# alpc91/SGRL

Hardware: AMD Instinct MI355X
Metric: env-steps/sec (whole node) + SET-actor fwd us/step, 3d_walker mix @8192 envs/GPU (higher is better)
Workload: dtype f64 (dynamics) / f32 (SET actor, obs); 1 GPU; 3D_Walker++ 8 variants x 1024 envs per GPU (config 3), random U(-1,1) actions, auto-reset, SET actor forward on every step, random-init weights; envs_per_gpu=8192, obs_max_len=287, action_max_len=21, replay_gather=none (single rank)

## Files before the change

include/sgrl_model.h:

```cpp
#ifndef SGRL_MODEL_H
#define SGRL_MODEL_H

#include <stdint.h>

#ifdef __HIPCC__
#define SGRL_HD __host__ __device__ inline
#else
#define SGRL_HD static inline
#endif

#define SGRL_MAGIC 0x5347524C
#define SGRL_MAXDEPTH 8

enum {
  SGRL_H_MAGIC = 0,
  SGRL_H_NBODY,
  SGRL_H_NJNT,
  SGRL_H_NQ,
  SGRL_H_NV,
  SGRL_H_NU,
  SGRL_H_NGEOM,
  SGRL_H_NPAIR,
  SGRL_H_INTEGRATOR,
  SGRL_H_FRAME_SKIP,
  SGRL_H_DONE_RULE,
  SGRL_H_TARGET_V2,
  SGRL_H_RESET_VEL_NORMAL,
  SGRL_H_NHEIGHT_BODIES,
  SGRL_H_HEIGHT_BODY0,
  SGRL_H_HEIGHT_BODY1,
  SGRL_H_MAX_ROWS,
  SGRL_H_PGS_ITERS,
  SGRL_H_SOLVER,
  SGRL_NHDR = 24
};

enum {
  SGRL_F_TIMESTEP = 0,
  SGRL_F_GRAV_X, SGRL_F_GRAV_Y, SGRL_F_GRAV_Z,
  SGRL_F_HEIGHT_LO, SGRL_F_HEIGHT_HI, SGRL_F_ANG_LIMIT,
  SGRL_F_ALIVE_BONUS, SGRL_F_HEADING_WEIGHT, SGRL_F_CTRL_COST,
  SGRL_F_RESET_POS_NOISE, SGRL_F_RESET_VEL_NOISE,
  SGRL_F_PGS_TOL,
  SGRL_F_TOTAL_MASS,
  SGRL_NFHDR = 16
};

enum {
  SGRL_RC_DMIN = 0, SGRL_RC_DMAX, SGRL_RC_WIDTH, SGRL_RC_MID, SGRL_RC_POWER,
  SGRL_RC_K, SGRL_RC_B, SGRL_RC_MARGIN, SGRL_RC_MU, SGRL_RC_TRAN, SGRL_RC_RF1, SGRL_RC_RF2,
  SGRL_ROWC = 12
};

enum { SGRL_GEOM_PLANE = 0, SGRL_GEOM_SPHERE = 2, SGRL_GEOM_CAPSULE = 3 };
enum { SGRL_JNT_FREE = 0, SGRL_JNT_HINGE = 3 };

#ifndef SGRL_CONST_AS
#define SGRL_CONST_AS
#endif
#ifndef SGRL_ITAB_AS
#define SGRL_ITAB_AS
#endif
#ifndef SGRL_FTAB_AS
#define SGRL_FTAB_AS
#endif
typedef const SGRL_CONST_AS int32_t* sgrl_hdr_t;
typedef const SGRL_CONST_AS double* sgrl_fhdr_t;
typedef const SGRL_ITAB_AS int32_t* sgrl_itab_t;
typedef const SGRL_FTAB_AS double* sgrl_ftab_t;

typedef struct SgrlModelView {
  sgrl_hdr_t hdr;
  sgrl_fhdr_t fhdr;
  int nbody, njnt, nq, nv, nu, ngeom, npair;
  sgrl_itab_t body_parent, body_jntadr, body_jntnum, body_dofadr, body_dofnum, body_limbtype;
  sgrl_itab_t jnt_type, jnt_body, jnt_qposadr, jnt_dofadr, jnt_limited;
  sgrl_itab_t dof_body, dof_jnt, dof_parent;
  sgrl_itab_t geom_type, geom_body;
  sgrl_itab_t pair_g1, pair_g2, pair_condim;
  sgrl_itab_t act_dof, act_slot;
  sgrl_itab_t body_depth;
  sgrl_itab_t body_path;
  sgrl_itab_t body_subend;
  sgrl_itab_t body_dofmask;
  sgrl_itab_t dof_act;
  sgrl_ftab_t qpos0;
  sgrl_ftab_t body_pos, body_quat, body_ipos, body_inertia, body_mass, body_invweight0;
  sgrl_ftab_t jnt_pos, jnt_axis, jnt_range, jnt_stiffness, jnt_solref, jnt_solimp, jnt_margin;
  sgrl_ftab_t dof_armature, dof_damping, dof_invweight0;
  sgrl_ftab_t geom_pos, geom_quat, geom_size;
  sgrl_ftab_t pair_mu, pair_margin, pair_solref, pair_solimp;
  sgrl_ftab_t act_gear, act_ctrlrange;
  sgrl_ftab_t geom_axis;
  sgrl_ftab_t pair_rowc;
  sgrl_ftab_t jnt_rowc;
  int n_int, n_f64;
} SgrlModelView;

SGRL_HD int sgrl_model_view_dims(const int32_t* dims, sgrl_hdr_t hdr_src, sgrl_fhdr_t fhdr_src, sgrl_itab_t ib, sgrl_ftab_t fb,
                                 SgrlModelView* v) {
  if (dims[SGRL_H_MAGIC] != SGRL_MAGIC) return -1;
  v->hdr = hdr_src;
  v->fhdr = fhdr_src;
  const int nb = dims[SGRL_H_NBODY], nj = dims[SGRL_H_NJNT], nq = dims[SGRL_H_NQ], nv = dims[SGRL_H_NV];
  const int nu = dims[SGRL_H_NU], ng = dims[SGRL_H_NGEOM], np = dims[SGRL_H_NPAIR];
  v->nbody = nb; v->njnt = nj; v->nq = nq; v->nv = nv; v->nu = nu; v->ngeom = ng; v->npair = np;
  sgrl_itab_t p = ib + SGRL_NHDR;
  v->body_parent = p; p += nb;
  v->body_jntadr = p; p += nb;
  v->body_jntnum = p; p += nb;
  v->body_dofadr = p; p += nb;
  v->body_dofnum = p; p += nb;
  v->body_limbtype = p; p += nb;
  v->jnt_type = p; p += nj;
  v->jnt_body = p; p += nj;
  v->jnt_qposadr = p; p += nj;
  v->jnt_dofadr = p; p += nj;
  v->jnt_limited = p; p += nj;
// ... 71 lines not shown
```

sgrl_amd/csrc/step_body.h:

```cpp
#pragma once

#include <math.h>
#include <stdint.h>

#include "../../include/sgrl_model.h"

#ifdef __HIPCC__
#define SGRL_DEV __device__ __forceinline__
#else
#define SGRL_DEV inline
#endif

namespace sgrl {

constexpr double kMinVal = 1e-15;
constexpr double kMinImp = 0.0001;
constexpr double kMaxImp = 0.9999;
constexpr double kPi = 3.14159265358979323846;
constexpr int kNAMax = 32;
constexpr int kBppMaxIter = 40;
constexpr int kSlabRows = 256;
constexpr int kPivotRows = 64;
constexpr int kPrevRows = 48;
constexpr int kSlabLdy = 47;
// ... 183 lines not shown
SGRL_DEV void quat2mat(double* m, const double* q) {
  const double q00 = q[0] * q[0], q11 = q[1] * q[1], q22 = q[2] * q[2], q33 = q[3] * q[3];
  m[0] = q00 + q11 - q22 - q33; m[4] = q00 - q11 + q22 - q33; m[8] = q00 - q11 - q22 + q33;
  m[1] = 2 * (q[1] * q[2] - q[0] * q[3]); m[2] = 2 * (q[1] * q[3] + q[0] * q[2]);
  m[3] = 2 * (q[1] * q[2] + q[0] * q[3]); m[5] = 2 * (q[2] * q[3] - q[0] * q[1]);
  m[6] = 2 * (q[1] * q[3] - q[0] * q[2]); m[7] = 2 * (q[2] * q[3] + q[0] * q[1]);
}
SGRL_DEV void mat_vec(double* r, const double* m, const double* v) {
  const double x = m[0] * v[0] + m[1] * v[1] + m[2] * v[2];
  const double y = m[3] * v[0] + m[4] * v[1] + m[5] * v[2];
  const double z = m[6] * v[0] + m[7] * v[1] + m[8] * v[2];
  r[0] = x; r[1] = y; r[2] = z;
}
SGRL_DEV void axisangle2quat(double* q, const double* axis, double angle) {
  if (angle == 0.0) { q[0] = 1; q[1] = 0; q[2] = 0; q[3] = 0; return; }
  double s, c;
  sincos(0.5 * angle, &s, &c);
  q[0] = c; q[1] = axis[0] * s; q[2] = axis[1] * s; q[3] = axis[2] * s;
}
SGRL_DEV void inert_mul(double* f, const double* I, const double* mv) {
  const double* w = mv; const double* v = mv + 3; const double* h = I + 6;
  double hv[3], hw[3];
  cross3(hv, h, v); cross3(hw, h, w);
  f[0] = I[0] * w[0] + I[3] * w[1] + I[4] * w[2] + hv[0];
  f[1] = I[3] * w[0] + I[1] * w[1] + I[5] * w[2] + hv[1];
  f[2] = I[4] * w[0] + I[5] * w[1] + I[2] * w[2] + hv[2];
  f[3] = I[9] * v[0] - hw[0]; f[4] = I[9] * v[1] - hw[1]; f[5] = I[9] * v[2] - hw[2];
}
SGRL_DEV void cross_motion(double* r, const double* vel, const double* m) {
  double a[3], b[3], c[3];
  cross3(a, vel, m); cross3(b, vel, m + 3); cross3(c, vel + 3, m);
  r[0] = a[0]; r[1] = a[1]; r[2] = a[2];
  r[3] = b[0] + c[0]; r[4] = b[1] + c[1]; r[5] = b[2] + c[2];
}
SGRL_DEV void cross_force(double* r, const double* vel, const double* f) {
  double a[3], b[3], c[3];
  cross3(a, vel, f); cross3(b, vel + 3, f + 3); cross3(c, vel, f + 3);
  r[0] = a[0] + b[0]; r[1] = a[1] + b[1]; r[2] = a[2] + b[2];
  r[3] = c[0]; r[4] = c[1]; r[5] = c[2];
}
SGRL_DEV void ld3(double* r, const double* p) { r[0] = p[0]; r[1] = p[1]; r[2] = p[2]; }
SGRL_DEV void ld6(double* r, const double* p) { r[0] = p[0]; r[1] = p[1]; r[2] = p[2]; r[3] = p[3]; r[4] = p[4]; r[5] = p[5]; }
SGRL_DEV int popcount64(uint64_t x) {
#ifdef __HIPCC__
  return __popcll(x);
#else
  return __builtin_popcountll(x);
#endif
}
SGRL_DEV int clz64(uint64_t x) {
#ifdef __HIPCC__
  return __clzll((long long)x);
#else
  return __builtin_clzll(x);
#endif
}
SGRL_DEV int tri(int i) { return i * (i + 1) / 2; }
SGRL_DEV void tri_decode(int p, int* a_out, int* b_out) {
  int a = (int)((sqrtf(8.0f * (float)p + 1.0f) - 1.0f) * 0.5f);
  a += ((a + 1) * (a + 2) / 2 <= p) ? 1 : 0;
  a -= (a * (a + 1) / 2 > p) ? 1 : 0;
  *a_out = a; *b_out = p - a * (a + 1) / 2;
}
SGRL_DEV bool dof_in_mask(sgrl_itab_t mask2, int d) {
  const uint32_t w = (uint32_t)(d < 32 ? mask2[0] : mask2[1]);
  return (w >> (d & 31)) & 1u;
}

SGRL_DEV double rng_uniform01(uint64_t seed, uint32_t env_id, uint32_t episode, uint32_t stream, uint32_t idx) {
  uint32_t c0 = idx >> 2, c1 = episode, c2 = stream, c3 = (uint32_t)(seed >> 32);
  uint32_t k0 = (uint32_t)seed, k1 = env_id;
  for (int r = 0; r < 10; r++) {
    const uint64_t p0 = (uint64_t)0xD2511F53u * c0, p1 = (uint64_t)0xCD9E8D57u * c2;
    const uint32_t n0 = (uint32_t)(p1 >> 32) ^ c1 ^ k0, n1 = (uint32_t)p1;
    const uint32_t n2 = (uint32_t)(p0 >> 32) ^ c3 ^ k1, n3 = (uint32_t)p0;
    c0 = n0; c1 = n1; c2 = n2; c3 = n3;
    k0 += 0x9E3779B9u; k1 += 0xBB67AE85u;
  }
  const uint32_t lane = idx & 3u;
  const uint32_t x = lane == 0 ? c0 : (lane == 1 ? c1 : (lane == 2 ? c2 : c3));
  return ((double)x + 0.5) * (1.0 / 4294967296.0);
}

#ifdef SGRL_PHASE_PROF
#define SGRL_TICK(id) w.tick(id)
#else
#define SGRL_TICK(id)
#endif

template <class W>
struct Engine {
  W& w;
  SgrlModelView m;
  const Layout& o;
  double* S;
  int32_t* I;
  double* big_scratch = nullptr;
  bool linv = false;

  SGRL_DEV Engine(W& w_, const SgrlModelView& m_, const Layout& o_, double* S_, int32_t* I_)
      : w(w_), m(m_), o(o_), S(S_), I(I_) {}

  SGRL_DEV void fence_view() {
    if (W::kFixedDims) return;
    m.body_parent = w.fenced(m.body_parent); m.body_jntadr = w.fenced(m.body_jntadr);
    m.body_jntnum = w.fenced(m.body_jntnum); m.body_dofadr = w.fenced(m.body_dofadr);
    m.body_dofnum = w.fenced(m.body_dofnum); m.body_limbtype = w.fenced(m.body_limbtype);
    m.jnt_type = w.fenced(m.jnt_type); m.jnt_body = w.fenced(m.jnt_body);
    m.jnt_qposadr = w.fenced(m.jnt_qposadr); m.jnt_dofadr = w.fenced(m.jnt_dofadr);
    m.jnt_limited = w.fenced(m.jnt_limited); m.dof_body = w.fenced(m.dof_body); m.dof_jnt = w.fenced(m.dof_jnt);
    m.dof_parent = w.fenced(m.dof_parent); m.geom_type = w.fenced(m.geom_type);
    m.geom_body = w.fenced(m.geom_body); m.pair_g1 = w.fenced(m.pair_g1); m.pair_g2 = w.fenced(m.pair_g2);
    m.pair_condim = w.fenced(m.pair_condim); m.act_dof = w.fenced(m.act_dof); m.act_slot = w.fenced(m.act_slot);
    m.body_depth = w.fenced(m.body_depth); m.body_path = w.fenced(m.body_path);
    m.body_subend = w.fenced(m.body_subend); m.body_dofmask = w.fenced(m.body_dofmask);
    m.dof_act = w.fenced(m.dof_act);
  }

  SGRL_DEV static void quat_rot(double* r, const double* q, const double* v) {
    double mtx[9];
    quat2mat(mtx, q);
    mat_vec(r, mtx, v);
  }

  SGRL_DEV void kinematics() {
    w.lanes(1, [&](int) {
      double q[4] = {S[o.qpos + 3], S[o.qpos + 4], S[o.qpos + 5], S[o.qpos + 6]};
      quat_normalize(q);
      S[o.qpos + 3] = q[0]; S[o.qpos + 4] = q[1]; S[o.qpos + 5] = q[2]; S[o.qpos + 6] = q[3];
    });
    const int TJ = o.Y, TB = o.Y + 17 * o.nj;
    w.lanes(o.nj, [&](int j) {
      if (m.jnt_type[j] == SGRL_JNT_FREE) return;
      double ja[3], ql[4];
      ld3(ja, m.jnt_axis + 3 * j);
      const int qa = m.jnt_qposadr[j];
      axisangle2quat(ql, ja, S[o.qpos + qa] - m.qpos0[qa]);
      double* t = S + TJ + 17 * j;
      for (int k = 0; k < 4; k++) t[k] = ql[k];
      for (int k = 0; k < 3; k++) { t[4 + k] = ja[k]; t[7 + k] = m.jnt_pos[3 * j + k]; }
    });
    w.lanes(o.nb, [&](int c) {
      if (c < 2) return;
      double p[3], q[4];
      ld3(p, m.body_pos + 3 * c);
      for (int k = 0; k < 4; k++) q[k] = m.body_quat[4 * c + k];
      const int j0 = m.body_jntadr[c], jn = m.body_jntnum[c];
      for (int j = j0; j < j0 + jn; j++) {
        double* t = S + TJ + 17 * j;
        double ql[4], jp[3], anchor[3], v[3], qn[4];
        for (int k = 0; k < 4; k++) ql[k] = t[k];
        ld3(jp, t + 7);
        quat_rot(v, q, jp);
        for (int k = 0; k < 3; k++) anchor[k] = p[k] + v[k];
        for (int k = 0; k < 4; k++) t[10 + k] = q[k];
        for (int k = 0; k < 3; k++) t[14 + k] = anchor[k];
        quat_mul(qn, q, ql);
        for (int k = 0; k < 4; k++) q[k] = qn[k];
        quat_rot(v, q, jp);
        for (int k = 0; k < 3; k++) p[k] = anchor[k] - v[k];
      }
      double* u = S + TB + 7 * c;
      for (int k = 0; k < 3; k++) u[k] = p[k];
      for (int k = 0; k < 4; k++) u[3 + k] = q[k];
    });
    w.lanes(o.nb, [&](int b) {
      if (b == 0) {
        for (int k = 0; k < 3; k++) S[o.xpos + k] = 0;
        S[o.xquat] = 1; S[o.xquat + 1] = 0; S[o.xquat + 2] = 0; S[o.xquat + 3] = 0;
        for (int k = 0; k < 9; k++) S[o.xmat + k] = (k % 4 == 0) ? 1.0 : 0.0;
        return;
      }
      double pos[3], quat[4], mat[9];
      const int depth = m.body_depth[b];
      for (int k = 0; k < 3; k++) pos[k] = S[o.qpos + k];
      for (int k = 0; k < 4; k++) quat[k] = S[o.qpos + 3 + k];
      quat_normalize(quat);
      for (int lvl = 1; lvl < depth; lvl++) {
        const int c = m.body_path[8 * b + lvl];
        const double* u = S + TB + 7 * c;
        double pl[3], qloc[4], t[3], qn[4];
        ld3(pl, u);
        for (int k = 0; k < 4; k++) qloc[k] = u[3 + k];
        quat_rot(t, quat, pl);
        for (int k = 0; k < 3; k++) pos[k] += t[k];
        quat_mul(qn, quat, qloc);
        for (int k = 0; k < 4; k++) quat[k] = qn[k];
      }
      quat_normalize(quat);
      quat2mat(mat, quat);
      for (int k = 0; k < 3; k++) S[o.xpos + 3 * b + k] = pos[k];
      for (int k = 0; k < 4; k++) S[o.xquat + 4 * b + k] = quat[k];
      for (int k = 0; k < 9; k++) S[o.xmat + 9 * b + k] = mat[k];
      double ip[3], t[3];
      ld3(ip, m.body_ipos + 3 * b);
      mat_vec(t, mat, ip);
      for (int k = 0; k < 3; k++) S[o.xipos + 3 * b + k] = pos[k] + t[k];
    });
    w.lanes(o.nj, [&](int j) {
      if (m.jnt_type[j] == SGRL_JNT_FREE) {
        const int b = m.jnt_body[j];
        for (int k = 0; k < 3; k++) { S[o.xanchor + 3 * j + k] = S[o.xpos + 3 * b + k]; S[o.xaxis + 3 * j + k] = (k == 2) ? 1.0 : 0.0; }
        return;
      }
      const int par = m.body_parent[m.jnt_body[j]];
      const double* t = S + TJ + 17 * j;
      double pp[3], qp[4], qb[4], ql[4], al[3], ja[3], v[3], ax[3];
      ld3(pp, S + o.xpos + 3 * par);
      for (int k = 0; k < 4; k++) { qp[k] = S[o.xquat + 4 * par + k]; ql[k] = t[10 + k]; }
      ld3(al, t + 14); ld3(ja, t + 4);
      quat_rot(v, qp, al);
      quat_mul(qb, qp, ql);
      quat_rot(ax, qb, ja);
      for (int k = 0; k < 3; k++) { S[o.xanchor + 3 * j + k] = pp[k] + v[k]; S[o.xaxis + 3 * j + k] = ax[k]; }
    });
  }

  SGRL_DEV void com_pos() {
    const double mt = m.fhdr[SGRL_F_TOTAL_MASS];
    double comr[3];
    for (int k = 0; k < 3; k++)
      comr[k] = w.sum(o.nb, [&](int b) { return b == 0 ? 0.0 : m.body_mass[b] * S[o.xipos + 3 * b + k]; }) / mt;
    w.lanes(o.nb > o.nv ? o.nb : o.nv, [&](int i) {
      const double com[3] = {comr[0], comr[1], comr[2]};
      if (i == 0) for (int k = 0; k < 3; k++) S[o.misc + MS_COM + k] = com[k];
      if (i >= 1 && i < o.nb) {
        const int b = i;
        double R[9], Wm[9], RI[9];
        for (int k = 0; k < 9; k++) R[k] = S[o.xmat + 9 * b + k];
        sgrl_ftab_t ib = m.body_inertia + 6 * b;
        const double Im[9] = {ib[0], ib[3], ib[4], ib[3], ib[1], ib[5], ib[4], ib[5], ib[2]};
        for (int r = 0; r < 3; r++)
// ... 146 lines not shown
  }
  SGRL_DEV void plane_sphere(int slot, double margin, const double* ppos, const double* n, const double* c, double r, const double* tangent) {
    const double d[3] = {c[0] - ppos[0], c[1] - ppos[1], c[2] - ppos[2]};
    const double dist = dot3(d, n) - r;
    double pos[3];
    for (int k = 0; k < 3; k++) pos[k] = c[k] - n[k] * (r + 0.5 * dist);
    put_contact(slot, dist < margin, dist, pos, n, tangent);
  }
  SGRL_DEV void collide() {
    w.lanes(o.np, [&](int p) {
      const int g1 = m.pair_g1[p], g2 = m.pair_g2[p];
      double p1[3], a1[3], p2[3], a2[3];
      geom_pose(g1, p1, a1); geom_pose(g2, p2, a2);
      const double margin = m.pair_margin[p];
      const int t1 = m.geom_type[g1], t2 = m.geom_type[g2];
      if (t1 == SGRL_GEOM_PLANE) {
        const double* n = a1;
        if (t2 == SGRL_GEOM_SPHERE) {
          plane_sphere(2 * p, margin, p1, n, p2, m.geom_size[3 * g2], nullptr);
          I[o.con_valid + 2 * p + 1] = 0;
        } else {
          const double* ax = a2;
          const double h = m.geom_size[3 * g2 + 1], r = m.geom_size[3 * g2];
          double ca[3], cb[3];
          for (int k = 0; k < 3; k++) { ca[k] = p2[k] + ax[k] * h; cb[k] = p2[k] - ax[k] * h; }
          plane_sphere(2 * p, margin, p1, n, ca, r, ax);
          plane_sphere(2 * p + 1, margin, p1, n, cb, r, ax);
        }
      } else {
        const double h1 = m.geom_size[3 * g1 + 1], h2 = m.geom_size[3 * g2 + 1];
        const double r1 = m.geom_size[3 * g1], r2 = m.geom_size[3 * g2];
        const double d[3] = {p1[0] - p2[0], p1[1] - p2[1], p1[2] - p2[2]};
        const double bb = dot3(a1, a2), c = dot3(a1, d), f = dot3(a2, d);
        const double den = 1.0 - bb * bb;
        const bool general = fabs(den) >= kMinVal;
        int made = 0;
        I[o.con_valid + 2 * p] = 0;
        I[o.con_valid + 2 * p + 1] = 0;
        for (int q = 0; q < (general ? 1 : 4) && made < 2; q++) {
          double s, t;
          if (general) {
            s = (bb * f - c) / den;
            if (s > h1) s = h1;
            if (s < -h1) s = -h1;
            t = bb * s + f;
            if (t > h2) { t = h2; s = bb * t - c; if (s > h1) s = h1; if (s < -h1) s = -h1; }
            else if (t < -h2) { t = -h2; s = bb * t - c; if (s > h1) s = h1; if (s < -h1) s = -h1; }
          } else if (q < 2) {
            s = q ? -h1 : h1; t = bb * s + f;
            if (t > h2) t = h2;
            if (t < -h2) t = -h2;
          } else {
            t = (q & 1) ? -h2 : h2; s = bb * t - c;
            if (s > h1) s = h1;
            if (s < -h1) s = -h1;
          }
          double c1[3], nn[3];
          for (int k = 0; k < 3; k++) { c1[k] = p1[k] + s * a1[k]; nn[k] = (p2[k] + t * a2[k]) - c1[k]; }
          const double len = sqrt(dot3(nn, nn));
          const double dist = len - r1 - r2;
          if (dist >= margin) continue;
          if (len < kMinVal) { nn[0] = 1; nn[1] = 0; nn[2] = 0; } else for (int k = 0; k < 3; k++) nn[k] /= len;
          double pos[3];
          for (int k = 0; k < 3; k++) pos[k] = c1[k] + nn[k] * (r1 + 0.5 * dist);
          put_contact(2 * p + made, true, dist, pos, nn, nullptr);
          made++;
        }
      }
    });
  }

  SGRL_DEV void bias_and_smooth_force() {
    w.lanes(o.nb, [&](int b) {
      if (b == 0) { for (int k = 0; k < 6; k++) S[o.cfrc + k] = 0; return; }
      double cv[6] = {0, 0, 0, 0, 0, 0};
      double ca[6] = {0, 0, 0, -m.fhdr[SGRL_F_GRAV_X], -m.fhdr[SGRL_F_GRAV_Y], -m.fhdr[SGRL_F_GRAV_Z]};
      const int depth = m.body_depth[b];
      for (int lvl = 0; lvl < depth; lvl++) {
        const int c = m.body_path[8 * b + lvl];
        const int j0 = m.body_jntadr[c], jn = m.body_jntnum[c];
        for (int j = j0; j < j0 + jn; j++) {
          const int d0 = m.jnt_dofadr[j];
          if (m.jnt_type[j] == SGRL_JNT_FREE) {
            for (int d = 0; d < 3; d++) {
              const double qv = S[o.qvel + d0 + d];
              for (int k = 0; k < 6; k++) cv[k] += S[o.cdof + 6 * (d0 + d) + k] * qv;
            }
            double cd[3][6], dd[6];
            for (int d = 0; d < 3; d++) ld6(cd[d], S + o.cdof + 6 * (d0 + 3 + d));
            for (int d = 0; d < 3; d++) {
              cross_motion(dd, cv, cd[d]);
              const double qv = S[o.qvel + d0 + 3 + d];
              for (int k = 0; k < 6; k++) ca[k] += dd[k] * qv;
            }
            for (int d = 0; d < 3; d++) {
              const double qv = S[o.qvel + d0 + 3 + d];
              for (int k = 0; k < 6; k++) cv[k] += cd[d][k] * qv;
            }
          } else {
            double cd[6], dd[6];
            ld6(cd, S + o.cdof + 6 * d0);
            cross_motion(dd, cv, cd);
            const double qv = S[o.qvel + d0];
            for (int k = 0; k < 6; k++) { ca[k] += dd[k] * qv; cv[k] += cd[k] * qv; }
          }
        }
      }
      double ci[10], f1[6], iv[6], f2[6];
      for (int k = 0; k < 10; k++) ci[k] = S[o.cinert + 10 * b + k];
      inert_mul(f1, ci, ca);
      inert_mul(iv, ci, cv);
      cross_force(f2, cv, iv);
      for (int k = 0; k < 6; k++) S[o.cfrc + 6 * b + k] = f1[k] + f2[k];
    });
    w.lanes(o.nv, [&](int d) {
      const int b = m.dof_body[d], e = m.body_subend[b];
      double f[6] = {0, 0, 0, 0, 0, 0}, cd[6];
      for (int c = b; c < e; c++)
        for (int k = 0; k < 6; k++) f[k] += S[o.cfrc + 6 * c + k];
      ld6(cd, S + o.cdof + 6 * d);
      const double bias = dot6(cd, f);
      const int j = m.dof_jnt[d];
      double passive = -m.dof_damping[d] * S[o.qvel + d];
      if (m.jnt_type[j] == SGRL_JNT_HINGE) {
        const int qa = m.jnt_qposadr[j];
        passive -= m.jnt_stiffness[j] * (S[o.qpos + qa] - m.qpos0[qa]);
      }
      double q = passive - bias;
      const int u = m.dof_act[d];
      if (u >= 0) {
        double c = S[o.ctrl + u];
        const double lo = m.act_ctrlrange[2 * u], hi = m.act_ctrlrange[2 * u + 1];
        if (c < lo) c = lo;
        if (c > hi) c = hi;
        q += m.act_gear[u] * c;
      }
      S[o.qfs + d] = q;
    });
  }

  SGRL_DEV double impedance(const double* rc, double x_raw) {
    const double dmin = rc[SGRL_RC_DMIN], dmax = rc[SGRL_RC_DMAX], width = rc[SGRL_RC_WIDTH], mid = rc[SGRL_RC_MID], power = rc[SGRL_RC_POWER];
    if (dmin == dmax || width <= kMinVal) return 0.5 * (dmin + dmax);
    const double x = fabs(x_raw) / width;
    if (x >= 1) return dmax;
    if (x <= 0) return dmin;
    double y;
    if (power == 1) y = x;
    else if (power == 2) y = (x <= mid) ? (x * x) / mid : 1 - ((1 - x) * (1 - x)) / (1 - mid);
    else if (x <= mid) y = pow(x, power) / pow(mid, power - 1);
    else y = 1 - pow(1 - x, power) / pow(1 - mid, power - 1);
    return dmin + y * (dmax - dmin);
  }

  struct Rows {
    double *Y, *eR, *earef, *eb, *ef, *eidg, *C;
    int32_t *kind, *src, *sub, *flist;
  };
  SGRL_DEV Rows rows_lds() const {
    return Rows{S + o.Y, S + o.eR, S + o.earef, S + o.eb, S + o.ef, S + o.eidg, S + o.dead,
                I + o.row_kind, I + o.row_src, I + o.row_sub, I + o.flist};
  }
  SGRL_DEV Rows rows_hbm() const {
    double* p = big_scratch;
    const int mr = o.maxrows;
    Rows r;
    r.C = p; p += kPivotRows * (kPivotRows + 1) / 2;
    r.Y = p; p += (mr + 1) * o.ldy;
    r.eR = p; p += mr; r.earef = p; p += mr; r.eb = p; p += mr; r.ef = p; p += mr;
// ... 9 lines not shown
      int c = 0;
      if (t < 2 * o.nj) {
        const int j = t >> 1, side = (t & 1) ? 1 : -1;
        if (m.jnt_limited[j]) {
          const double q = S[o.qpos + m.jnt_qposadr[j]];
          const double dist = side * (m.jnt_range[2 * j + (side + 1) / 2] - q);
          if (dist < m.jnt_margin[j]) c = 1;
        }
      } else {
        const int sl = t - 2 * o.nj;
        if (I[o.con_valid + sl]) { const int dim = m.pair_condim[sl >> 1]; c = (dim == 1) ? 1 : 2 * (dim - 1); }
      }
      I[o.ecnt + t] = c;
    });
    if (nitem <= 64) {
      int total = 0;
      for (int k = 0; k < 4; k++) {
        cbits[k] = w.ballot(nitem, [&](int t) { return ((I[o.ecnt + t] >> k) & 1) != 0; });
        total += popcount64(cbits[k]) << k;
      }
      return total;
    }
    return (int)w.sum(nitem, [&](int t) { return (double)I[o.ecnt + t]; });
  }
  uint64_t cbits[4] = {0, 0, 0, 0};

  SGRL_DEV void fill_rows(const Rows& R, int wanted_total, int cap) {
    const int nitem = 2 * o.nj + o.ncon;
    if (wanted_total <= cap) {
      w.lanes(nitem, [&](int t) {
        int pre = 0;
        if (nitem <= 64) {
          const uint64_t below = (1ull << t) - 1;
          for (int k = 0; k < 4; k++) pre += popcount64(cbits[k] & below) << k;
        } else {
          for (int u = 0; u < t; u++) pre += I[o.ecnt + u];
        }
        const int c = I[o.ecnt + t];
        if (t == 0) { I[o.icnt + IC_NROW_WANTED] = wanted_total; I[o.icnt + IC_NROW] = wanted_total; }
        for (int k = 0; k < c; k++) {
          if (t < 2 * o.nj) { R.kind[pre] = (t & 1) ? ROW_LIMIT_HI : ROW_LIMIT_LO; R.src[pre] = t >> 1; R.sub[pre] = 0; }
          else { R.kind[pre + k] = (c == 1) ? ROW_CON1 : ROW_PYR; R.src[pre + k] = t - 2 * o.nj; R.sub[pre + k] = k; }
        }
      });
      return;
    }
    w.lanes(1, [&](int) {
      int nrow = 0, wanted = 0;
      const int maxrows = cap;
      for (int j = 0; j < o.nj; j++) {
        if (!m.jnt_limited[j]) continue;
        const double q = S[o.qpos + m.jnt_qposadr[j]];
        for (int side = -1; side <= 1; side += 2) {
          const double dist = side * (m.jnt_range[2 * j + (side + 1) / 2] - q);
          if (dist >= m.jnt_margin[j]) continue;
          wanted++;
          if (nrow >= maxrows) continue;
          R.kind[nrow] = side < 0 ? ROW_LIMIT_LO : ROW_LIMIT_HI;
          R.src[nrow] = j; R.sub[nrow] = 0;
          nrow++;
        }
      }
      for (int s = 0; s < o.ncon; s++) {
        if (!I[o.con_valid + s]) continue;
        const int p = s >> 1, dim = m.pair_condim[p];
        const int nr = (dim == 1) ? 1 : 2 * (dim - 1);
        wanted += nr;
        if (nrow + nr > maxrows) continue;
        for (int k = 0; k < nr; k++) {
          R.kind[nrow] = dim == 1 ? ROW_CON1 : ROW_PYR;
          R.src[nrow] = s; R.sub[nrow] = k;
          nrow++;
        }
      }
      I[o.icnt + IC_NROW] = nrow; I[o.icnt + IC_NROW_WANTED] = wanted;
      if (wanted > nrow) I[o.icnt + IC_OVERFLOW] += 1;
    });
  }

  template <bool BIG>
  SGRL_DEV void build_rows_and_halfsolve(const Rows& R) {
    const int nv = o.nv, ldy = o.ldy;
    const int nrow = I[o.icnt + IC_NROW];
    w.lanes(nrow + 1, [&](int r) {
      double* Yr = R.Y + r * ldy;
      if (r == nrow) {
        for (int d = 0; d < nv; d++) Yr[d] = S[o.qfs + d];
        return;
      }
      const int kind = R.kind[r], src = R.src[r], sub = R.sub[r];
      const bool lim = kind == ROW_LIMIT_LO || kind == ROW_LIMIT_HI;
      sgrl_ftab_t rcp = lim ? m.jnt_rowc + SGRL_ROWC * src : m.pair_rowc + SGRL_ROWC * (src >> 1);
      double rc[SGRL_ROWC];
      for (int k = 0; k < SGRL_ROWC; k++) rc[k] = rcp[k];
      double dist, vel;
      if (lim) {
        const int j = src, side = kind == ROW_LIMIT_LO ? -1 : 1, dof = m.jnt_dofadr[j];
        for (int d = 0; d < nv; d++) Yr[d] = 0;
        Yr[dof] = -side;
        const double q = S[o.qpos + m.jnt_qposadr[j]];
        dist = side * (m.jnt_range[2 * j + (side + 1) / 2] - q);
        vel = -side * S[o.qvel + dof];
      } else {
        const int s = src, p = s >> 1;
        const int b1 = m.geom_body[m.pair_g1[p]], b2 = m.geom_body[m.pair_g2[p]];
        const double mu = rc[SGRL_RC_MU];
        dist = S[o.con_dist + s];
        double off[3], dir[3];
        const double* fr = S + o.con_frame + o.fstride * s;
        for (int k = 0; k < 3; k++) off[k] = S[o.con_pos + 3 * s + k] - S[o.misc + MS_COM + k];
        if (kind == ROW_CON1) {
          for (int k = 0; k < 3; k++) dir[k] = fr[k];
        } else {
          const double sg = (sub & 1) ? -mu : mu;
          double tg[3];
          if (sub >> 1) cross3(tg, fr, fr + 3);
          else ld3(tg, fr + 3);
          for (int k = 0; k < 3; k++) dir[k] = fr[k] + sg * tg[k];
        }
        sgrl_itab_t mk1 = m.body_dofmask + 2 * b1;
        sgrl_itab_t mk2 = m.body_dofmask + 2 * b2;
        vel = 0;
        for (int d = 0; d < nv; d++) {
          double sgn = 0;
          if (b2 > 0 && dof_in_mask(mk2, d)) sgn += 1.0;
          if (b1 > 0 && dof_in_mask(mk1, d)) sgn -= 1.0;
          double val = 0;
          if (sgn != 0) {
            double cd[6], v[3];
            ld6(cd, S + o.cdof + 6 * d);
            cross3(v, cd, off);
            v[0] += cd[3]; v[1] += cd[4]; v[2] += cd[5];
            val = sgn * dot3(dir, v);
          }
          Yr[d] = val;
          vel += val * S[o.qvel + d];
        }
      }
      const bool pyr = kind == ROW_PYR;
      const double x = dist - rc[SGRL_RC_MARGIN];
      const double imp = impedance(rc, x);
      double Rreg = (1 - imp) / imp * (pyr ? rc[SGRL_RC_RF1] : rc[SGRL_RC_TRAN]);
      if (Rreg < kMinVal) Rreg = kMinVal;
      if (pyr) {
        Rreg = rc[SGRL_RC_RF2] * Rreg;
        if (Rreg < kMinVal) Rreg = kMinVal;
      }
      const double aref = -rc[SGRL_RC_B] * vel - rc[SGRL_RC_K] * imp * x;
      R.eR[r] = Rreg; R.earef[r] = aref;
      const int key = (kind << 16) | (src << 3) | sub;
      double f0 = 0;
      const int pn = I[o.icnt + IC_PREV_N];
      const int pcap = o.prevcap, pl = pn < pcap ? pn : pcap;
      bool hit = false;
      if (r < pl) {
        if (I[o.prev_key + r] == key) { f0 = S[o.prev_f + r]; hit = true; }
      } else if (r < pn) {
        const double* hf = big_scratch + slab_prev_offset(o.maxrows, o.ldy);
        const int32_t* hk = reinterpret_cast<const int32_t*>(hf + o.maxrows);
        if (hk[r] == key) { f0 = hf[r]; hit = true; }
      }
      if (!hit) {
        for (int k = 0; k < pl; k++) if (I[o.prev_key + k] == key) f0 = S[o.prev_f + k];
        if (pn > pcap) {
          const double* hf = big_scratch + slab_prev_offset(o.maxrows, o.ldy);
          const int32_t* hk = reinterpret_cast<const int32_t*>(hf + o.maxrows);
          for (int k = pcap; k < pn; k++) if (hk[k] == key) f0 = hf[k];
        }
      }
      R.ef[r] = f0;
    });
    SGRL_TICK(6);
    if (linv) {
      if (BIG || !w.trmm_rows(nrow + 1, nv, S + o.L, R.Y, ldy))
      w.lanes(nrow + 1, [&](int r) {
        double* Yr = R.Y + r * ldy;
        for (int d = nv - 1; d >= 0; d--) {
          const double* Ld = S + o.L + tri(d);
          double s0 = 0, s1 = 0, s2 = 0, s3 = 0;
          int c = 0;
          for (; c + 4 <= d + 1; c += 4) {
            const double a0 = Ld[c], a1 = Ld[c + 1], a2 = Ld[c + 2], a3 = Ld[c + 3];
            const double b0 = Yr[c], b1 = Yr[c + 1], b2 = Yr[c + 2], b3 = Yr[c + 3];
            s0 += a0 * b0; s1 += a1 * b1; s2 += a2 * b2; s3 += a3 * b3;
          }
          for (; c <= d; c++) s0 += Ld[c] * Yr[c];
          Yr[d] = (s0 + s1) + (s2 + s3);
        }
      });
    } else {
      w.trsm_lower_rows(nrow + 1, nv, S + o.L, S + o.dinv, R.Y, ldy);
    }
    SGRL_TICK(9);
    w.lanes(nrow > nv ? nrow : nv, [&](int r) {
      if (r < nrow) {
        const double* Yr = R.Y + r * ldy;
        const double* ys = R.Y + nrow * ldy;
        double q0 = 0, q1 = 0, t0 = 0, t1 = 0;
        int d = 0;
        for (; d + 2 <= nv; d += 2) {
          const double y0 = Yr[d], y1 = Yr[d + 1];
          q0 += y0 * y0; q1 += y1 * y1; t0 += y0 * ys[d]; t1 += y1 * ys[d + 1];
        }
        for (; d < nv; d++) { q0 += Yr[d] * Yr[d]; t0 += Yr[d] * ys[d]; }
        const double Rr = R.eR[r];
// ... 537 lines not shown
```

sgrl_amd/model_pack.py:

```python
import numpy as np

from . import mjcf
from .env_spec import env_spec_for

NHDR = 24
NFHDR = 16
(H_MAGIC, H_NBODY, H_NJNT, H_NQ, H_NV, H_NU, H_NGEOM, H_NPAIR, H_INTEGRATOR, H_FRAME_SKIP, H_DONE_RULE,
 H_TARGET_V2, H_RESET_VEL_NORMAL, H_NHEIGHT_BODIES, H_HEIGHT_BODY0, H_HEIGHT_BODY1, H_MAX_ROWS,
 H_PGS_ITERS, H_SOLVER) = range(19)
(F_TIMESTEP, F_GRAV_X, F_GRAV_Y, F_GRAV_Z, F_HEIGHT_LO, F_HEIGHT_HI, F_ANG_LIMIT, F_ALIVE_BONUS,
 F_HEADING_WEIGHT, F_CTRL_COST, F_RESET_POS_NOISE, F_RESET_VEL_NOISE, F_PGS_TOL, F_TOTAL_MASS) = range(14)

DEFAULT_MAX_ROWS = 48
DEFAULT_PGS_ITERS = 300
DEFAULT_PGS_TOL = 1e-10
DEFAULT_SOLVER = 1


MAXDEPTH = 8


def _derived_int_tables(model):
    nb, nv = model.nbody, model.nv
    depth = np.zeros(nb, dtype=np.int32)
    path = np.full((nb, MAXDEPTH), -1, dtype=np.int32)
    subend = np.zeros(nb, dtype=np.int32)
    mask = np.zeros((nb, 2), dtype=np.int32)
    for b in range(1, nb):
        chain = []
        a = b
        while a > 0:
            chain.append(a)
            a = int(model.body_parent[a])
        chain.reverse()
        if len(chain) > MAXDEPTH:
            raise ValueError("kinematic chain deeper than %d" % MAXDEPTH)
        depth[b] = len(chain)
        path[b, :len(chain)] = chain
        bits = 0
        for c in chain:
            for d in range(int(model.body_dofadr[c]), int(model.body_dofadr[c]) + int(model.body_dofnum[c])):
                bits |= 1 << d
        lo, hi = bits & 0xFFFFFFFF, (bits >> 32) & 0xFFFFFFFF
        mask[b] = np.array([lo, hi], dtype=np.uint32).view(np.int32)
    for b in range(nb - 1, 0, -1):
        subend[b] = max(subend[b], b + 1)
        p = int(model.body_parent[b])
        if p > 0:
            subend[p] = max(subend[p], subend[b])
    for b in range(1, nb):
        for c in range(b + 1, nb):
            inside = c < subend[b]
            a = c
            anc = False
            while a > 0:
                if a == b:
                    anc = True
                a = int(model.body_parent[a])
            if inside != anc:
                raise ValueError("bodies are not in pre-order")
    if nv > 64:
        raise ValueError("nv > 64 unsupported")
    dof_act = np.full(nv, -1, dtype=np.int32)
    for u in range(model.nu):
        dof_act[int(model.act_dof[u])] = u
    return [depth, path.ravel(), subend, mask.ravel(), dof_act]


ROWC = 12
MIN_IMP, MAX_IMP = 0.0001, 0.9999


def _row_constants(solref, solimp, margin, mu, tran, timestep):
    dmin, dmax, width, mid, power = (float(x) for x in solimp)
    dmin = min(max(dmin, MIN_IMP), MAX_IMP)
    dmax = min(max(dmax, MIN_IMP), MAX_IMP)
    width = max(width, 0.0)
    mid = min(max(mid, MIN_IMP), MAX_IMP)
    power = max(power, 1.0)
    tc, dr = max(float(solref[0]), 2 * float(timestep)), float(solref[1])
    k = 1.0 / (dmax * dmax * tc * tc * dr * dr)
    b = 2.0 / (dmax * tc)
    mu, tran = float(mu), float(tran)
    return [dmin, dmax, width, mid, power, k, b, float(margin), mu, tran, tran + mu * mu * tran, 2 * mu * mu]


def _derived_f64_tables(model):
    ng, npair, nj = model.ngeom, model.npair, model.njnt
    gq = np.asarray(model.geom_quat, dtype=np.float64).reshape(ng, 4)
    axis = np.empty((ng, 3))
    axis[:, 0] = 2 * (gq[:, 1] * gq[:, 3] + gq[:, 0] * gq[:, 2])
    axis[:, 1] = 2 * (gq[:, 2] * gq[:, 3] - gq[:, 0] * gq[:, 1])
    axis[:, 2] = gq[:, 0] * gq[:, 0] - gq[:, 1] * gq[:, 1] - gq[:, 2] * gq[:, 2] + gq[:, 3] * gq[:, 3]
    iw_body = np.asarray(model.body_invweight0, dtype=np.float64).reshape(-1, 2)
    iw_dof = np.asarray(model.dof_invweight0, dtype=np.float64).ravel()
    p_solref = np.asarray(model.pair_solref, dtype=np.float64).reshape(npair, 2)
    p_solimp = np.asarray(model.pair_solimp, dtype=np.float64).reshape(npair, 5)
    pair = np.zeros((npair, ROWC))
    for p in range(npair):
        b1 = int(model.geom_body[int(model.pair_g1[p])])
        b2 = int(model.geom_body[int(model.pair_g2[p])])
        pair[p] = _row_constants(p_solref[p], p_solimp[p], np.ravel(model.pair_margin)[p], np.ravel(model.pair_mu)[p],
                                 iw_body[b1, 0] + iw_body[b2, 0], model.timestep)
    j_solref = np.asarray(model.jnt_solref, dtype=np.float64).reshape(nj, 2)
    j_solimp = np.asarray(model.jnt_solimp, dtype=np.float64).reshape(nj, 5)
    jnt = np.zeros((nj, ROWC))
    for j in range(nj):
        jnt[j] = _row_constants(j_solref[j], j_solimp[j], np.ravel(model.jnt_margin)[j], 0.0,
                                iw_dof[int(model.jnt_dofadr[j])], model.timestep)
    return [axis.ravel(), pair.ravel(), jnt.ravel()]


def worst_case_rows(model):
    rows = int(np.sum(np.asarray(model.jnt_limited) != 0))
    for k in range(model.npair):
        g2 = int(model.pair_g2[k])
        ncon = 2 if (int(model.geom_type[int(model.pair_g1[k])]) == mjcf.GEOM_PLANE and int(model.geom_type[g2]) == mjcf.GEOM_CAPSULE) else 1
        dim = int(model.pair_condim[k])
        rows += ncon * (1 if dim == 1 else 2 * (dim - 1))
    return rows


def pack_model(model, spec=None, env_name=None, max_rows=DEFAULT_MAX_ROWS, pgs_iters=DEFAULT_PGS_ITERS,
               pgs_tol=DEFAULT_PGS_TOL, solver=DEFAULT_SOLVER):
    if spec is None:
        spec = env_spec_for(env_name or model.name)
    hdr = np.zeros(NHDR, dtype=np.int32)
    hdr[H_MAGIC] = mjcf.MAGIC
    hdr[H_NBODY], hdr[H_NJNT], hdr[H_NQ], hdr[H_NV] = model.nbody, model.njnt, model.nq, model.nv
    hdr[H_NU], hdr[H_NGEOM], hdr[H_NPAIR] = model.nu, model.ngeom, model.npair
    hdr[H_INTEGRATOR] = model.integrator
    hdr[H_FRAME_SKIP] = spec.frame_skip
    hdr[H_DONE_RULE] = spec.done_rule
    hdr[H_TARGET_V2] = 1 if spec.target_v2 else 0
    hdr[H_RESET_VEL_NORMAL] = 1 if spec.reset_vel_normal else 0
    hb = [model.body_names.index(n) for n in spec.height_bodies if n in model.body_names]
    hdr[H_NHEIGHT_BODIES] = len(hb)
    for i, b in enumerate(hb[:2]):
        hdr[H_HEIGHT_BODY0 + i] = b
    hdr[H_MAX_ROWS] = min(int(max_rows), max(1, worst_case_rows(model)))
    hdr[H_PGS_ITERS] = pgs_iters
    hdr[H_SOLVER] = solver
    ints = [hdr]
    for k in mjcf.Model.INT_FIELDS:
        ints.append(np.asarray(getattr(model, k), dtype=np.int32).ravel())
    ints.extend(_derived_int_tables(model))
    fh = np.zeros(NFHDR, dtype=np.float64)
    fh[F_TIMESTEP] = model.timestep
    fh[F_GRAV_X:F_GRAV_Z + 1] = model.gravity
    fh[F_HEIGHT_LO], fh[F_HEIGHT_HI], fh[F_ANG_LIMIT] = spec.height_lo, spec.height_hi, spec.ang_limit
    fh[F_ALIVE_BONUS], fh[F_HEADING_WEIGHT], fh[F_CTRL_COST] = spec.alive_bonus, spec.heading_weight, spec.ctrl_cost
    fh[F_RESET_POS_NOISE], fh[F_RESET_VEL_NOISE] = spec.reset_pos_noise, spec.reset_vel_noise
    fh[F_PGS_TOL] = pgs_tol
    fh[F_TOTAL_MASS] = float(np.sum(model.body_mass[1:]))
    fls = [fh]
    for k in mjcf.Model.F64_FIELDS:
        fls.append(np.asarray(getattr(model, k), dtype=np.float64).ravel())
    fls.extend(_derived_f64_tables(model))
    return np.ascontiguousarray(np.concatenate(ints)), np.ascontiguousarray(np.concatenate(fls))
```

sgrl_amd/vec_env.py:

```python
import collections.abc
import ctypes

import numpy as np

from . import _lib, mjcf, model_pack
from .env_spec import env_spec_for


class Box(object):

    def __init__(self, low, high, shape=None, dtype=np.float32):
        if shape is None:
            shape = np.shape(low)
        self.low = np.full(shape, low, dtype=dtype) if np.isscalar(low) else np.asarray(low, dtype=dtype)
        self.high = np.full(shape, high, dtype=dtype) if np.isscalar(high) else np.asarray(high, dtype=dtype)
        self.shape = tuple(shape)
        self.dtype = np.dtype(dtype)

    def sample(self):
        return np.random.uniform(self.low, self.high).astype(self.dtype)


class StepInfos(collections.abc.Sequence):
    __slots__ = ("_dist", "_trunc", "_extra")

    def __init__(self, dist, trunc, extra=None):
        self._dist, self._trunc, self._extra = dist, trunc, extra

    def __len__(self):
        return int(self._dist.shape[0])

    def __getitem__(self, i):
        if isinstance(i, slice):
            return tuple(self[j] for j in range(*i.indices(len(self))))
        n = len(self)
        if i < 0:
            i += n
        if not 0 <= i < n:
            raise IndexError(i)
        d = {"dist": float(self._dist[i])}
        if self._trunc[i]:
            d["TimeLimit.truncated"] = True
        if self._extra and i in self._extra:
            d.update(self._extra[i])
        return d

    def __eq__(self, other):
        if isinstance(other, (list, tuple, StepInfos)):
            return len(other) == len(self) and all(a == b for a, b in zip(self, other))
        return NotImplemented

    def __repr__(self):
        return "StepInfos(n=%d)" % len(self)


def _round_up(x, a=256):
    return (x + a - 1) // a * a


class VecEnv(object):

    def __init__(self, num_envs, observation_space, action_space):
        self.num_envs = num_envs
        self.observation_space = observation_space
        self.action_space = action_space

    def step(self, actions):
        self.step_async(actions)
        return self.step_wait()


def resolve_models(env_names, xml_paths=None):
    models = []
    for i, name in enumerate(env_names):
        if xml_paths is not None and xml_paths[i] is not None:
            models.append(mjcf.compile_mjcf(xml_paths[i], name=name.replace("_v2_", "_")))
        else:
            models.append(mjcf.load_asset(name.replace("_v2_", "_")))
    return models


class BatchedModularVecEnv(VecEnv):
    def __init__(self, env_names, envs_per_morph, obs_max_len=None, seed=0, device=None, max_episode_steps=1000,
                 xml_paths=None, env_id_base=0, max_rows=None,
                 pgs_iters=model_pack.DEFAULT_PGS_ITERS, pgs_tol=model_pack.DEFAULT_PGS_TOL,
                 solver=model_pack.DEFAULT_SOLVER):
        import torch
        self.torch = torch
        if not torch.cuda.is_available():
            raise _lib.SgrlError("BatchedModularVecEnv needs an MI355X: torch.cuda.is_available() is False "
                                 "(the engine has no CPU fallback)")
        self.device = torch.device(device if device is not None else "cuda:0")
        torch.cuda.set_device(self.device)
        self.env_names = list(env_names)
        counts = [envs_per_morph] * len(env_names) if np.isscalar(envs_per_morph) else list(envs_per_morph)
        assert len(counts) == len(env_names)
        self.counts = [int(c) for c in counts]
        self.models = resolve_models(self.env_names, xml_paths)
        self.num_limbs = [m.num_limbs for m in self.models]
        max_limbs = max(self.num_limbs)
        self.obs_max_len = int(obs_max_len) if obs_max_len else 41 * max_limbs
        self.action_max_len = 3 * max_limbs
        self.limb_obs_size, self.limb_action_size, self.max_action = 41, 3, 1.0
        n = sum(self.counts)
        self.env_morph = np.repeat(np.arange(len(env_names)), self.counts)
        self.morph_slices = []
        off = 0
        for c in self.counts:
            self.morph_slices.append(slice(off, off + c))
            off += c
        L0 = self.num_limbs[0]
        VecEnv.__init__(self, n, Box(-np.inf, np.inf, (41 * L0,), np.float64), Box(-1.0, 1.0, (3 * (L0 - 1),), np.float32))
        self.waiting = False
        self.closed = False
        rows_of = lambda m: max_rows if max_rows is not None else _lib.default_max_rows(m)
        self._blobs = [model_pack.pack_model(m, spec=env_spec_for(nm), max_rows=rows_of(m), pgs_iters=pgs_iters,
                                             pgs_tol=pgs_tol, solver=solver) for m, nm in zip(self.models, self.env_names)]
        L = _lib.lib()
        k = len(self._blobs)
        ibp = (ctypes.POINTER(ctypes.c_int32) * k)(*[b[0].ctypes.data_as(ctypes.POINTER(ctypes.c_int32)) for b in self._blobs])
        fbp = (ctypes.POINTER(ctypes.c_double) * k)(*[b[1].ctypes.data_as(ctypes.POINTER(ctypes.c_double)) for b in self._blobs])
        ibl = (ctypes.c_int32 * k)(*[len(b[0]) for b in self._blobs])
        fbl = (ctypes.c_int32 * k)(*[len(b[1]) for b in self._blobs])
        cnt = (ctypes.c_int32 * k)(*self.counts)
        h = ctypes.c_void_p()
        _lib.check(L.sgrl_engine_create(k, ibp, ibl, fbp, fbl, cnt, self.obs_max_len, self.action_max_len,
                                        ctypes.c_uint64(int(seed)), ctypes.c_uint32(int(env_id_base)),
                                        int(max_episode_steps), ctypes.byref(h)), "sgrl_engine_create")
        self._h = h
        self._L = L
        self.stride = L.sgrl_record_stride(h)
        self.lds_bytes = L.sgrl_lds_bytes(h)
        self.launch_groups = L.sgrl_launch_groups(h)
        self.fixed_dim_groups = L.sgrl_fixed_dim_groups(h)
        self.paired_envs = L.sgrl_paired_envs(h)
        dev = self.device
        secs = [("obs", 4 * n * self.obs_max_len), ("rew", 4 * n), ("dist", 4 * n), ("done", n), ("trunc", n)]
        self._out_off, off = {}, 0
        for name, nbytes in secs:
            self._out_off[name] = (off, nbytes)
            off += _round_up(nbytes)
        self._out = torch.zeros(off, dtype=torch.uint8, device=dev)
        sec = lambda name: self._out[self._out_off[name][0]:self._out_off[name][0] + self._out_off[name][1]]
        self.obs = sec("obs").view(torch.float32).view(n, self.obs_max_len)
        self.rew = sec("rew").view(torch.float32)
        self.dist = sec("dist").view(torch.float32)
        self.done = sec("done")
        self.trunc = sec("trunc")
        self._act = torch.zeros((n, self.action_max_len), dtype=torch.float32, device=dev)
        self._act_host = None
        self._fetch_event = torch.cuda.Event()
        self.obs64 = None
        self.rew64 = None
        self._overflow_seen = np.zeros(n, dtype=np.int64)
        self.overflow_check_every, self._steps_since_overflow_check = 16, 0

    def _stream(self):
        return ctypes.c_void_p(self.torch.cuda.current_stream(self.device).cuda_stream)

    def enable_f64_outputs(self):
        t = self.torch
        self.obs64 = t.zeros((self.num_envs, self.obs_max_len), dtype=t.float64, device=self.device)
        self.rew64 = t.zeros(self.num_envs, dtype=t.float64, device=self.device)

    def _p(self, t):
        return ctypes.c_void_p(0 if t is None else t.data_ptr())

    def reset_device(self):
        _lib.check(self._L.sgrl_reset(self._h, self._p(self.obs), self._p(self.obs64), self._stream()), "sgrl_reset")
        return self.obs

    def step_device(self, actions, auto_reset=True):
        assert actions.is_cuda and actions.dtype == self.torch.float32 and actions.is_contiguous()
        assert tuple(actions.shape) == (self.num_envs, self.action_max_len)
        _lib.check(self._L.sgrl_step(self._h, self._p(actions), self._p(self.obs), self._p(self.rew), self._p(self.done),
                                     self._p(self.dist), self._p(self.trunc), self._p(self.obs64), self._p(self.rew64),
                                     int(bool(auto_reset)), self._stream()), "sgrl_step")
        return self.obs, self.rew, self.done, self.dist

    def time_steps(self, actions, reps):
        ms = ctypes.c_float(0)
        _lib.check(self._L.sgrl_time_steps(self._h, self._p(actions), self._p(self.obs), self._p(self.rew),
                                           self._p(self.done), int(reps), self._stream(), ctypes.byref(ms)),
                   "sgrl_time_steps")
        return float(ms.value)

    def get_records(self):
        rec = np.zeros((self.num_envs, self.stride))
        cnt = np.zeros((self.num_envs, 4), dtype=np.int32)
        _lib.check(self._L.sgrl_get_records(self._h, ctypes.c_void_p(rec.ctypes.data), ctypes.c_void_p(cnt.ctypes.data)),
                   "sgrl_get_records")
        return rec, cnt

    def set_records(self, rec, cnt=None):
        rec = np.ascontiguousarray(rec, dtype=np.float64)
        assert rec.shape == (self.num_envs, self.stride)
        cp = None
        if cnt is not None:
            cnt = np.ascontiguousarray(cnt, dtype=np.int32)
            cp = ctypes.c_void_p(cnt.ctypes.data)
# ... 117 lines not shown
```

Before: 2.022 million env-steps/s.

## Specialize kinematics and contact row build on per-model structure flags

Adds a structure bitfield to the model header, computed at pack time: hinge anchors at zero, identity body quats, and a support flag. The kernel uses it to skip anchor rotation in forward kinematics, and to add only the linear free-joint velocity directly instead of a full cdof multiply. Contact Jacobian rows are filled by walking only the set bits of the two bodies' dof masks instead of testing every dof. These cut per-env arithmetic and branching in the dynamics step, at the cost of extra specialized code paths whose correctness depends on the pack-time flags.

```diff
diff --git a/include/sgrl_model.h b/include/sgrl_model.h
--- a/include/sgrl_model.h
+++ b/include/sgrl_model.h
@@ -32,8 +32,11 @@
   SGRL_H_MAX_ROWS,
   SGRL_H_PGS_ITERS,
   SGRL_H_SOLVER,
+  SGRL_H_STRUCT,
   SGRL_NHDR = 24
 };
+
+enum { SGRL_ST_ANCHOR0 = 1, SGRL_ST_QUAT_ID = 2, SGRL_ST_SUPPORT = 4 };
 
 enum {
   SGRL_F_TIMESTEP = 0,
diff --git a/sgrl_amd/csrc/step_body.h b/sgrl_amd/csrc/step_body.h
--- a/sgrl_amd/csrc/step_body.h
+++ b/sgrl_amd/csrc/step_body.h
@@ -289,6 +289,10 @@
   return ((double)x + 0.5) * (1.0 / 4294967296.0);
 }
 
+#ifndef SGRL_STRUCT_ITEMS
+#define SGRL_STRUCT_ITEMS 15
+#endif
+
 #ifdef SGRL_PHASE_PROF
 #define SGRL_TICK(id) w.tick(id)
 #else
@@ -324,6 +328,8 @@
     m.dof_act = w.fenced(m.dof_act);
   }
 
+  SGRL_DEV bool structure(int bit) const { return (W::hdr_const(m, SGRL_H_STRUCT) & SGRL_STRUCT_ITEMS & bit) != 0; }
+
   SGRL_DEV static void quat_rot(double* r, const double* q, const double* v) {
     double mtx[9];
     quat2mat(mtx, q);
@@ -337,6 +343,7 @@
       S[o.qpos + 3] = q[0]; S[o.qpos + 4] = q[1]; S[o.qpos + 5] = q[2]; S[o.qpos + 6] = q[3];
     });
     const int TJ = o.Y, TB = o.Y + 17 * o.nj;
+    const bool anchor0 = structure(SGRL_ST_ANCHOR0);
     w.lanes(o.nj, [&](int j) {
       if (m.jnt_type[j] == SGRL_JNT_FREE) return;
       double ja[3], ql[4];
@@ -345,7 +352,8 @@
       axisangle2quat(ql, ja, S[o.qpos + qa] - m.qpos0[qa]);
       double* t = S + TJ + 17 * j;
       for (int k = 0; k < 4; k++) t[k] = ql[k];
-      for (int k = 0; k < 3; k++) { t[4 + k] = ja[k]; t[7 + k] = m.jnt_pos[3 * j + k]; }
+      for (int k = 0; k < 3; k++) t[4 + k] = ja[k];
+      if (!anchor0) for (int k = 0; k < 3; k++) t[7 + k] = m.jnt_pos[3 * j + k];
     });
     w.lanes(o.nb, [&](int c) {
       if (c < 2) return;
@@ -355,6 +363,15 @@
       const int j0 = m.body_jntadr[c], jn = m.body_jntnum[c];
       for (int j = j0; j < j0 + jn; j++) {
         double* t = S + TJ + 17 * j;
+        if (anchor0) {
+          for (int k = 0; k < 4; k++) t[10 + k] = q[k];
+          for (int k = 0; k < 3; k++) t[14 + k] = p[k];
+          double ql[4], qn[4];
+          for (int k = 0; k < 4; k++) ql[k] = t[k];
+          quat_mul(qn, q, ql);
+          for (int k = 0; k < 4; k++) q[k] = qn[k];
+          continue;
+        }
         double ql[4], jp[3], anchor[3], v[3], qn[4];
         for (int k = 0; k < 4; k++) ql[k] = t[k];
         ld3(jp, t + 7);
@@ -667,9 +684,13 @@
         for (int j = j0; j < j0 + jn; j++) {
           const int d0 = m.jnt_dofadr[j];
           if (m.jnt_type[j] == SGRL_JNT_FREE) {
-            for (int d = 0; d < 3; d++) {
-              const double qv = S[o.qvel + d0 + d];
-              for (int k = 0; k < 6; k++) cv[k] += S[o.cdof + 6 * (d0 + d) + k] * qv;
+            if (SGRL_STRUCT_ITEMS & 8) {
+              for (int d = 0; d < 3; d++) cv[3 + d] += S[o.qvel + d0 + d];
+            } else {
+              for (int d = 0; d < 3; d++) {
+                const double qv = S[o.qvel + d0 + d];
+                for (int k = 0; k < 6; k++) cv[k] += S[o.cdof + 6 * (d0 + d) + k] * qv;
+              }
             }
             double cd[3][6], dd[6];
             for (int d = 0; d < 3; d++) ld6(cd[d], S + o.cdof + 6 * (d0 + 3 + d));
@@ -845,6 +866,7 @@
   SGRL_DEV void build_rows_and_halfsolve(const Rows& R) {
     const int nv = o.nv, ldy = o.ldy;
     const int nrow = I[o.icnt + IC_NROW];
+    const bool support = structure(SGRL_ST_SUPPORT);
     w.lanes(nrow + 1, [&](int r) {
       double* Yr = R.Y + r * ldy;
       if (r == nrow) {
@@ -857,9 +879,10 @@
       double rc[SGRL_ROWC];
       for (int k = 0; k < SGRL_ROWC; k++) rc[k] = rcp[k];
       double dist, vel;
+      if (support) for (int d = 0; d < nv; d++) Yr[d] = 0;
       if (lim) {
         const int j = src, side = kind == ROW_LIMIT_LO ? -1 : 1, dof = m.jnt_dofadr[j];
-        for (int d = 0; d < nv; d++) Yr[d] = 0;
+        if (!support) for (int d = 0; d < nv; d++) Yr[d] = 0;
         Yr[dof] = -side;
         const double q = S[o.qpos + m.jnt_qposadr[j]];
         dist = side * (m.jnt_range[2 * j + (side + 1) / 2] - q);
@@ -884,6 +907,30 @@
         sgrl_itab_t mk1 = m.body_dofmask + 2 * b1;
         sgrl_itab_t mk2 = m.body_dofmask + 2 * b2;
         vel = 0;
+        if (support) {
+          auto walk = [&](auto plus, auto bits) {
+            while (bits) {
+              const int d = sizeof(bits) == 8 ? __builtin_ctzll(bits) : __builtin_ctz((uint32_t)bits);
+              const double sgn = ((plus >> d) & 1) ? 1.0 : -1.0;
+              bits &= bits - 1;
+              double cd[6], v[3];
+              ld6(cd, S + o.cdof + 6 * d);
+              cross3(v, cd, off);
+              v[0] += cd[3]; v[1] += cd[4]; v[2] += cd[5];
+              const double val = sgn * dot3(dir, v);
+              Yr[d] = val;
+              vel += val * S[o.qvel + d];
+            }
+          };
+          if (nv <= 32) {
+            const uint32_t m1 = b1 > 0 ? (uint32_t)mk1[0] : 0u, m2 = b2 > 0 ? (uint32_t)mk2[0] : 0u;
+            walk(m2 & ~m1, m1 ^ m2);
+          } else {
+            const uint64_t m1 = b1 > 0 ? ((uint32_t)mk1[0] | ((uint64_t)(uint32_t)mk1[1] << 32)) : 0ull;
+            const uint64_t m2 = b2 > 0 ? ((uint32_t)mk2[0] | ((uint64_t)(uint32_t)mk2[1] << 32)) : 0ull;
+            walk(m2 & ~m1, m1 ^ m2);
+          }
+        } else
         for (int d = 0; d < nv; d++) {
           double sgn = 0;
           if (b2 > 0 && dof_in_mask(mk2, d)) sgn += 1.0;
diff --git a/sgrl_amd/model_pack.py b/sgrl_amd/model_pack.py
--- a/sgrl_amd/model_pack.py
+++ b/sgrl_amd/model_pack.py
@@ -7,7 +7,7 @@
 NFHDR = 16
 (H_MAGIC, H_NBODY, H_NJNT, H_NQ, H_NV, H_NU, H_NGEOM, H_NPAIR, H_INTEGRATOR, H_FRAME_SKIP, H_DONE_RULE,
  H_TARGET_V2, H_RESET_VEL_NORMAL, H_NHEIGHT_BODIES, H_HEIGHT_BODY0, H_HEIGHT_BODY1, H_MAX_ROWS,
- H_PGS_ITERS, H_SOLVER) = range(19)
+ H_PGS_ITERS, H_SOLVER, H_STRUCT) = range(20)
 (F_TIMESTEP, F_GRAV_X, F_GRAV_Y, F_GRAV_Z, F_HEIGHT_LO, F_HEIGHT_HI, F_ANG_LIMIT, F_ALIVE_BONUS,
  F_HEADING_WEIGHT, F_CTRL_COST, F_RESET_POS_NOISE, F_RESET_VEL_NOISE, F_PGS_TOL, F_TOTAL_MASS) = range(14)
 
@@ -18,6 +18,7 @@
 
 
 MAXDEPTH = 8
+ST_ANCHOR0, ST_QUAT_ID, ST_SUPPORT = 1, 2, 4
 
 
 def _derived_int_tables(model):
@@ -65,6 +66,18 @@
     for u in range(model.nu):
         dof_act[int(model.act_dof[u])] = u
     return [depth, path.ravel(), subend, mask.ravel(), dof_act]
+
+
+def structure_flags(model):
+    hinge = np.asarray(model.jnt_type).ravel() == mjcf.JNT_HINGE
+    jp = np.asarray(model.jnt_pos, dtype=np.float64).reshape(-1, 3)
+    bq = np.asarray(model.body_quat, dtype=np.float64).reshape(-1, 4)
+    flags = 0
+    if np.all(jp[hinge] == 0.0):
+        flags |= ST_ANCHOR0
+    if np.all(bq == np.array([1.0, 0.0, 0.0, 0.0])):
+        flags |= ST_QUAT_ID
+    return flags
 
 
 ROWC = 12
@@ -122,7 +135,7 @@
 
 
 def pack_model(model, spec=None, env_name=None, max_rows=DEFAULT_MAX_ROWS, pgs_iters=DEFAULT_PGS_ITERS,
-               pgs_tol=DEFAULT_PGS_TOL, solver=DEFAULT_SOLVER):
+               pgs_tol=DEFAULT_PGS_TOL, solver=DEFAULT_SOLVER, structure=True):
     if spec is None:
         spec = env_spec_for(env_name or model.name)
     hdr = np.zeros(NHDR, dtype=np.int32)
@@ -145,6 +158,8 @@
     for k in mjcf.Model.INT_FIELDS:
         ints.append(np.asarray(getattr(model, k), dtype=np.int32).ravel())
     ints.extend(_derived_int_tables(model))
+    if structure:
+        hdr[H_STRUCT] = structure_flags(model) | ST_SUPPORT
     fh = np.zeros(NFHDR, dtype=np.float64)
     fh[F_TIMESTEP] = model.timestep
     fh[F_GRAV_X:F_GRAV_Z + 1] = model.gravity
diff --git a/sgrl_amd/vec_env.py b/sgrl_amd/vec_env.py
--- a/sgrl_amd/vec_env.py
+++ b/sgrl_amd/vec_env.py
@@ -84,7 +84,7 @@
     def __init__(self, env_names, envs_per_morph, obs_max_len=None, seed=0, device=None, max_episode_steps=1000,
                  xml_paths=None, env_id_base=0, max_rows=None,
                  pgs_iters=model_pack.DEFAULT_PGS_ITERS, pgs_tol=model_pack.DEFAULT_PGS_TOL,
-                 solver=model_pack.DEFAULT_SOLVER):
+                 solver=model_pack.DEFAULT_SOLVER, structure=True):
         import torch
         self.torch = torch
         if not torch.cuda.is_available():
@@ -115,7 +115,7 @@
         self.closed = False
         rows_of = lambda m: max_rows if max_rows is not None else _lib.default_max_rows(m)
         self._blobs = [model_pack.pack_model(m, spec=env_spec_for(nm), max_rows=rows_of(m), pgs_iters=pgs_iters,
-                                             pgs_tol=pgs_tol, solver=solver) for m, nm in zip(self.models, self.env_names)]
+                                             pgs_tol=pgs_tol, solver=solver, structure=structure) for m, nm in zip(self.models, self.env_names)]
         L = _lib.lib()
         k = len(self._blobs)
         ibp = (ctypes.POINTER(ctypes.c_int32) * k)(*[b[0].ctypes.data_as(ctypes.POINTER(ctypes.c_int32)) for b in self._blobs])
```

Measured after the change: 2.042 million env-steps/s, median of 6. About the same (+1.0%).
